# parthjaggi/flow

Measured on AMD Instinct MI355X. Metric: env-steps/sec, higher is better.
Workload: dtype mixed

## Files before the change

### flow_amd/csrc/flowsim_pair.h

```cpp
#pragma once
#include "flowsim_kernels.h"

namespace fs {

typedef float f2 __attribute__((ext_vector_type(2)));
typedef unsigned u2v __attribute__((__vector_size__(8)));

enum : int { DPP_ROW_NEWBCAST0 = 0x150, DPP_ROW_NEWBCAST8 = 0x158 };

__device__ __forceinline__ f2 fma2(f2 a, f2 b, f2 c) { return __builtin_elementwise_fma(a, b, c); }
__device__ __forceinline__ f2 splat(float a) { return f2{a, a}; }

__device__ __forceinline__ f2 pk_mul(f2 a, f2 b) { return a * b; }
__device__ __forceinline__ f2 pk_add(f2 a, f2 b) { return a + b; }
__device__ __forceinline__ f2 pk_sub(f2 a, f2 b) { return a - b; }
__device__ __forceinline__ f2 pk_fma(f2 a, f2 b, f2 c) { return fma2(a, b, c); }
__device__ __forceinline__ f2 pk_fnma(f2 a, f2 b, f2 c) { return fma2(-a, b, c); }
__device__ __forceinline__ float nonneg_else(float x, float y) {
  const unsigned a = __builtin_bit_cast(unsigned, x), b = __builtin_bit_cast(unsigned, y);
  return __builtin_bit_cast(float, min(a, b));
}

template <int ROW>
__device__ __forceinline__ float next_a(float v, bool last, int lane) {
// ... 70 lines not shown
  f2 adt, ddt;
};
template <bool FASTDIV>
__device__ __forceinline__ f2 sumo_acc_pair(f2 v, f2 vl, f2 h, const SumoPair& c, f2 one) {
  f2 gap;
  gap.x = tmax(h.x, 1e-3f);
  gap.y = tmax(h.y, 1e-3f);
  const f2 num = pk_mul(v, pk_sub(v, vl));
  const f2 dq = div_const2<FASTDIV>(num, c.ts, c.rc_ts);
  const f2 dyn = pk_add(pk_mul(v, c.tau), dq);
  f2 ss;
  ss.x = tmax(0.0f, dyn.x);
  ss.y = tmax(0.0f, dyn.y);
  ss = pk_add(c.min_gap, ss);
  const f2 q = FASTDIV ? div_core2(ss, gap, one) : f2{ss.x / gap.x, ss.y / gap.y};
  const f2 r = div_const2<FASTDIV>(v, c.smax, c.rc_smax);
  const f2 r2 = pk_mul(r, r);
  return pk_mul(c.maxa, pk_sub(pk_sub(one, pk_mul(r2, r2)), pk_mul(q, q)));
}

struct PairConsts {
  f2 p0, p1, p2, p5, rc_v0, tsab, rc_ab, one, dt2, ramp2, L2, rc_L2, len_lead, gap2, vmask, tvm;
  float c1e3;
  double ms64, rc_ms64;
  unsigned long long last_mask;
};
#define FS_PAIR_A_NAME pair_step_asm_a
#define FS_PAIR_A_NZ 0
#define FS_PAIR_A_NZ_PARAM
#include "flowsim_pair_step_a.inc"
#undef FS_PAIR_A_NAME
#undef FS_PAIR_A_NZ
#undef FS_PAIR_A_NZ_PARAM
#define FS_PAIR_A_NAME pair_step_asm_a_nz
#define FS_PAIR_A_NZ 1
#define FS_PAIR_A_NZ_PARAM , f2 nz
#include "flowsim_pair_step_a.inc"
#undef FS_PAIR_A_NAME
#undef FS_PAIR_A_NZ
#undef FS_PAIR_A_NZ_PARAM
#define FS_PAIR_A_NAME pair_step_asm_a_sm
#define FS_PAIR_A_NZ 0
#define FS_PAIR_A_NZ_PARAM
#include "flowsim_pair_step_a_sm.inc"
#undef FS_PAIR_A_NAME
#undef FS_PAIR_A_NZ
#undef FS_PAIR_A_NZ_PARAM
// ... 9 lines not shown
  asm volatile(
      "v_sub_f32_e32 v118, v112, v113\n"
      "v_sub_f32_e32 v132, v115, v114\n"
      "v_subrev_f32_dpp v119, v112, v113 row_shl:1 row_mask:0xf bank_mask:0xf bound_ctrl:1\n"
      "v_subrev_f32_dpp v134, v112, v113 row_newbcast:0 row_mask:0xf bank_mask:0xf\n"
      "v_sub_f32_dpp v133, v114, v115 row_shl:1 row_mask:0xf bank_mask:0xf bound_ctrl:1\n"
      "v_sub_f32_dpp v135, v114, v115 row_newbcast:0 row_mask:0xf bank_mask:0xf\n"
      "v_cndmask_b32_e64 v119, v119, v134, %[last]\n"
      "v_cndmask_b32_e64 v133, v133, v135, %[last]\n"
      "v_pk_add_f32 v[126:127], v[132:133], %[L2]\n"
      "v_min_u32_e32 v132, v132, v126\n"
      "v_min_u32_e32 v133, v133, v127\n"
      "v_pk_add_f32 v[116:117], v[132:133], %[lenlead] neg_lo:[0,1] neg_hi:[0,1]\n"
      "v_pk_add_f32 v[126:127], v[116:117], %[gap2] neg_lo:[0,1] neg_hi:[0,1]\n"
      "v_min_f32_e32 v126, v126, v127\n"
      "v_alignbit_b32 %[cb], %[cb], v126, 31\n"
      "v_pk_fma_f32 v[124:125], v[112:113], %[vmask], %[tvm]\n"
      "v_pk_mul_f32 v[124:125], v[124:125], v[124:125]\n"
      "v_add_f32_e32 %[sq], v124, v125\n"
      "v_cvt_f64_f32_e32 v[130:131], v112\n"
      "v_cvt_f64_f32_e32 v[132:133], v113\n"
      "v_mul_f64 v[134:135], v[130:131], %[rcms]\n"
      "v_mul_f64 v[136:137], v[132:133], %[rcms]\n"
      "v_fma_f64 v[130:131], -v[134:135], %[ms], v[130:131]\n"
      "v_fma_f64 v[132:133], -v[136:137], %[ms], v[132:133]\n"
      "v_fma_f64 v[134:135], v[130:131], %[rcms], v[134:135]\n"
      "v_fma_f64 v[136:137], v[132:133], %[rcms], v[136:137]\n"
      "v_cvt_f32_f64_e32 v128, v[134:135]\n"
      "v_cvt_f32_f64_e32 v129, v[136:137]\n"
      : "+{v[112:113]}"(V), "+{v[114:115]}"(X), "+{v[116:117]}"(H), "+{v[118:119]}"(DVL), "={v[128:129]}"(OV),
        [cb] "+v"(crash_bits), [sq] "=&v"(sq)
      : [L2] "v"(c.L2), [lenlead] "v"(c.len_lead), [gap2] "v"(c.gap2), [vmask] "v"(c.vmask), [tvm] "v"(c.tvm),
        [ms] "v"(c.ms64), [rcms] "v"(c.rc_ms64), [last] "s"(c.last_mask)
      : "v124", "v125", "v126", "v127", "v130", "v131", "v132", "v133", "v134", "v135", "v136", "v137");
}

struct MixedConsts {
  f2 p0, p1, p2, p5, rc_v0, tsab, rc_ab, one, gap2, vmask, tvm;
  float c1e3;
  double dt, ramp, L, rc_L, rc_ms, len_b, len_next, zero;
  unsigned L_lo, L_hi, thr;
  unsigned long long last_mask;
};
__device__ __forceinline__ void mixed_step_asm_a(f2& V32, double& XA, double& XB, double& VA, double& VB, f2& H, f2& DVL,
                                                 f2& OV, const MixedConsts& c) {
  asm volatile(
      "v_pk_mul_f32 v[124:125], v[112:113], v[142:143]\n"
      "v_pk_mul_f32 v[126:127], v[124:125], %[rcab]\n"
      "v_pk_fma_f32 v[130:131], v[126:127], %[tsab], v[124:125] neg_lo:[1,0,0] neg_hi:[1,0,0]\n"
      "v_pk_fma_f32 v[126:127], v[130:131], %[rcab], v[126:127]\n"
      "v_pk_mul_f32 v[124:125], v[112:113], %[rcv0]\n"
      "v_rcp_f32_e32 v122, v140\n"
      "v_rcp_f32_e32 v123, v141\n"
      "v_pk_fma_f32 v[130:131], v[124:125], %[p0], v[112:113] neg_lo:[1,0,0] neg_hi:[1,0,0]\n"
      "v_pk_fma_f32 v[124:125], v[130:131], %[rcv0], v[124:125]\n"
      "v_pk_mul_f32 v[130:131], v[112:113], %[p1]\n"
      "v_pk_add_f32 v[130:131], v[130:131], v[126:127]\n"
      "v_pk_fma_f32 v[126:127], v[140:141], v[122:123], %[one] neg_lo:[1,0,0] neg_hi:[1,0,0]\n"
      "v_max_f32_e32 v130, 0, v130\n"
      "v_max_f32_e32 v131, 0, v131\n"
      "v_pk_fma_f32 v[122:123], v[126:127], v[122:123], v[122:123]\n"
      "v_pk_add_f32 v[130:131], %[p5], v[130:131]\n"
      "v_pk_mul_f32 v[124:125], v[124:125], v[124:125]\n"
      "v_pk_mul_f32 v[126:127], v[130:131], v[122:123]\n"
      "v_pk_mul_f32 v[124:125], v[124:125], v[124:125]\n"
      "v_pk_fma_f32 v[132:133], v[140:141], v[126:127], v[130:131] neg_lo:[1,0,0] neg_hi:[1,0,0]\n"
      "v_pk_add_f32 v[124:125], %[one], v[124:125] neg_lo:[0,1] neg_hi:[0,1]\n"
      "v_pk_fma_f32 v[126:127], v[132:133], v[122:123], v[126:127]\n"
      "v_pk_fma_f32 v[132:133], v[140:141], v[126:127], v[130:131] neg_lo:[1,0,0] neg_hi:[1,0,0]\n"
      "v_pk_fma_f32 v[126:127], v[132:133], v[122:123], v[126:127]\n"
      "v_pk_mul_f32 v[126:127], v[126:127], v[126:127]\n"
      "v_pk_add_f32 v[124:125], v[124:125], v[126:127] neg_lo:[0,1] neg_hi:[0,1]\n"
      "v_pk_mul_f32 v[124:125], %[p2], v[124:125]\n"
      "v_cvt_f64_f32_e32 v[130:131], v124\n"
      "v_cvt_f64_f32_e32 v[132:133], v125\n"
      "v_mul_f64 v[130:131], v[130:131], %[dt]\n"
      "v_mul_f64 v[132:133], v[132:133], %[dt]\n"
      "v_add_f64 v[130:131], v[118:119], v[130:131]\n"
      "v_add_f64 v[132:133], v[138:139], v[132:133]\n"
      "v_max_f64 v[130:131], v[130:131], %[zero]\n"
      "v_max_f64 v[132:133], v[132:133], %[zero]\n"
      "v_add_f64 v[130:131], v[130:131], -v[118:119]\n"
      "v_add_f64 v[132:133], v[132:133], -v[138:139]\n"
      "v_mul_f64 v[130:131], v[130:131], %[ramp]\n"
      "v_mul_f64 v[132:133], v[132:133], %[ramp]\n"
      "v_add_f64 v[118:119], v[118:119], v[130:131]\n"
      "v_add_f64 v[138:139], v[138:139], v[132:133]\n"
      "v_cvt_f32_f64_e32 v112, v[118:119]\n"
      "v_cvt_f32_f64_e32 v113, v[138:139]\n"
      "v_mul_f64 v[130:131], v[118:119], %[dt]\n"
      "v_mul_f64 v[132:133], v[138:139], %[dt]\n"
      "v_add_f64 v[114:115], v[114:115], v[130:131]\n"
      "v_add_f64 v[116:117], v[116:117], v[132:133]\n"
      "v_mul_f64 v[120:121], v[118:119], %[rcms]\n"
      "v_mul_f64 v[122:123], v[138:139], %[rcms]\n"
      "v_cvt_f32_f64_e32 v128, v[120:121]\n"
      "v_cvt_f32_f64_e32 v129, v[122:123]\n"
      : "+{v[112:113]}"(V32), "+{v[114:115]}"(XA), "+{v[116:117]}"(XB), "+{v[118:119]}"(VA), "+{v[138:139]}"(VB),
        "+{v[140:141]}"(H), "+{v[142:143]}"(DVL), "={v[128:129]}"(OV)
      : [rcab] "v"(c.rc_ab), [tsab] "v"(c.tsab), [rcv0] "v"(c.rc_v0), [p0] "v"(c.p0), [p1] "v"(c.p1), [p2] "v"(c.p2),
        [p5] "v"(c.p5), [one] "v"(c.one), [dt] "v"(c.dt), [ramp] "v"(c.ramp), [rcms] "v"(c.rc_ms), [zero] "v"(c.zero)
      : "v120", "v121", "v122", "v123", "v124", "v125", "v126", "v127", "v130", "v131", "v132", "v133");
}
struct MixedSumoConsts { double fl0a, fl0b, adta, adtb, ddta, ddtb; };
__device__ __forceinline__ void mixed_step_asm_a_sm(f2& V32, double& XA, double& XB, double& VA, double& VB, f2& H,
                                                    f2& DVL, f2& OV, const MixedConsts& c, const SumoPair& m,
                                                    const MixedSumoConsts& d) {
  asm volatile(
      "v_pk_mul_f32 v[124:125], v[112:113], v[142:143]\n"
      "v_pk_mul_f32 v[126:127], v[124:125], %[rcab]\n"
      "v_pk_mul_f32 v[150:151], v[124:125], %[rcts]\n"
      "v_pk_fma_f32 v[130:131], v[126:127], %[tsab], v[124:125] neg_lo:[1,0,0] neg_hi:[1,0,0]\n"
      "v_pk_fma_f32 v[152:153], v[150:151], %[ts], v[124:125] neg_lo:[1,0,0] neg_hi:[1,0,0]\n"
      "v_pk_fma_f32 v[126:127], v[130:131], %[rcab], v[126:127]\n"
      "v_pk_fma_f32 v[150:151], v[152:153], %[rcts], v[150:151]\n"
      "v_max_f32_e32 v146, v140, %[c1e3]\n"
// ... 32 lines not shown
      "v_pk_fma_f32 v[134:135], v[146:147], v[152:153], v[150:151] neg_lo:[1,0,0] neg_hi:[1,0,0]\n"
      "v_pk_add_f32 v[124:125], %[one], v[124:125] neg_lo:[0,1] neg_hi:[0,1]\n"
      "v_pk_add_f32 v[154:155], %[one], v[154:155] neg_lo:[0,1] neg_hi:[0,1]\n"
      "v_pk_fma_f32 v[126:127], v[132:133], v[122:123], v[126:127]\n"
      "v_pk_fma_f32 v[152:153], v[134:135], v[148:149], v[152:153]\n"
      "v_pk_fma_f32 v[132:133], v[140:141], v[126:127], v[130:131] neg_lo:[1,0,0] neg_hi:[1,0,0]\n"
      "v_pk_fma_f32 v[134:135], v[146:147], v[152:153], v[150:151] neg_lo:[1,0,0] neg_hi:[1,0,0]\n"
      "v_pk_fma_f32 v[126:127], v[132:133], v[122:123], v[126:127]\n"
      "v_pk_fma_f32 v[152:153], v[134:135], v[148:149], v[152:153]\n"
      "v_pk_mul_f32 v[126:127], v[126:127], v[126:127]\n"
      "v_pk_mul_f32 v[152:153], v[152:153], v[152:153]\n"
      "v_pk_add_f32 v[124:125], v[124:125], v[126:127] neg_lo:[0,1] neg_hi:[0,1]\n"
      "v_pk_add_f32 v[154:155], v[154:155], v[152:153] neg_lo:[0,1] neg_hi:[0,1]\n"
      "v_pk_mul_f32 v[124:125], %[p2], v[124:125]\n"
      "v_pk_mul_f32 v[154:155], %[maxa], v[154:155]\n"
      "v_cvt_f64_f32_e32 v[130:131], v124\n"
      "v_cvt_f64_f32_e32 v[132:133], v125\n"
      "v_cvt_f64_f32_e32 v[134:135], v154\n"
      "v_cvt_f64_f32_e32 v[136:137], v155\n"
      "v_mul_f64 v[130:131], v[130:131], %[dt]\n"
      "v_mul_f64 v[132:133], v[132:133], %[dt]\n"
      "v_mul_f64 v[134:135], v[134:135], %[dt]\n"
      "v_mul_f64 v[136:137], v[136:137], %[dt]\n"
      "v_add_f64 v[130:131], v[118:119], v[130:131]\n"
      "v_add_f64 v[132:133], v[138:139], v[132:133]\n"
      "v_add_f64 v[134:135], v[118:119], v[134:135]\n"
      "v_add_f64 v[136:137], v[138:139], v[136:137]\n"
      "v_max_f64 v[130:131], v[130:131], %[zero]\n"
      "v_max_f64 v[132:133], v[132:133], %[zero]\n"
      "v_max_f64 v[134:135], v[134:135], %[fl0a]\n"
      "v_max_f64 v[136:137], v[136:137], %[fl0b]\n"
      "v_add_f64 v[130:131], v[130:131], -v[118:119]\n"
      "v_add_f64 v[132:133], v[132:133], -v[138:139]\n"
      "v_mul_f64 v[130:131], v[130:131], %[ramp]\n"
      "v_mul_f64 v[132:133], v[132:133], %[ramp]\n"
      "v_add_f64 v[130:131], v[118:119], v[130:131]\n"
      "v_add_f64 v[132:133], v[138:139], v[132:133]\n"
      "v_min_f64 v[130:131], v[130:131], v[134:135]\n"
      "v_min_f64 v[132:133], v[132:133], v[136:137]\n"
      "v_add_f64 v[134:135], v[118:119], %[adta]\n"
      "v_add_f64 v[136:137], v[138:139], %[adtb]\n"
      "v_min_f64 v[130:131], v[130:131], v[134:135]\n"
      "v_min_f64 v[132:133], v[132:133], v[136:137]\n"
      "v_add_f64 v[134:135], v[118:119], -%[ddta]\n"
      "v_add_f64 v[136:137], v[138:139], -%[ddtb]\n"
      "v_max_f64 v[118:119], v[130:131], v[134:135]\n"
      "v_max_f64 v[138:139], v[132:133], v[136:137]\n"
      "v_cvt_f32_f64_e32 v112, v[118:119]\n"
      "v_cvt_f32_f64_e32 v113, v[138:139]\n"
      "v_mul_f64 v[130:131], v[118:119], %[dt]\n"
      "v_mul_f64 v[132:133], v[138:139], %[dt]\n"
      "v_add_f64 v[114:115], v[114:115], v[130:131]\n"
      "v_add_f64 v[116:117], v[116:117], v[132:133]\n"
      "v_mul_f64 v[120:121], v[118:119], %[rcms]\n"
      "v_mul_f64 v[122:123], v[138:139], %[rcms]\n"
      "v_cvt_f32_f64_e32 v128, v[120:121]\n"
      "v_cvt_f32_f64_e32 v129, v[122:123]\n"
      : "+{v[112:113]}"(V32), "+{v[114:115]}"(XA), "+{v[116:117]}"(XB), "+{v[118:119]}"(VA), "+{v[138:139]}"(VB),
        "+{v[140:141]}"(H), "+{v[142:143]}"(DVL), "={v[128:129]}"(OV)
      : [c1e3] "v"(c.c1e3), [rcab] "v"(c.rc_ab), [tsab] "v"(c.tsab), [rcv0] "v"(c.rc_v0), [p0] "v"(c.p0),
        [p1] "v"(c.p1), [p2] "v"(c.p2), [p5] "v"(c.p5), [one] "v"(c.one), [dt] "v"(c.dt), [ramp] "v"(c.ramp),
        [rcms] "v"(c.rc_ms), [zero] "v"(c.zero), [rcts] "v"(m.rc_ts), [ts] "v"(m.ts),
        [rcsm] "v"(m.rc_smax), [smax] "v"(m.smax), [tau] "v"(m.tau), [mgap] "v"(m.min_gap), [maxa] "v"(m.maxa),
        [fl0a] "v"(d.fl0a), [fl0b] "v"(d.fl0b), [adta] "v"(d.adta), [adtb] "v"(d.adtb), [ddta] "v"(d.ddta),
        [ddtb] "v"(d.ddtb)
      : "v120", "v121", "v122", "v123", "v124", "v125", "v126", "v127", "v130", "v131", "v132", "v133", "v134",
        "v135", "v136", "v137", "v146", "v147", "v148", "v149", "v150", "v151", "v152", "v153", "v154", "v155");
}
__device__ __forceinline__ void mixed_step_asm_b(f2& V32, double& XA, double& XB, f2& H, f2& DVL, f2& OX, const double& WA,
                                                 const double& WB, float& ct, float& sq, unsigned long long& need,
                                                 const MixedConsts& c) {
  asm volatile(
      "v_sub_f32_e32 v142, v112, v113\n"
      "v_subrev_f32_dpp v143, v112, v113 row_shl:1 row_mask:0xf bank_mask:0xf bound_ctrl:1\n"
      "v_subrev_f32_dpp v124, v112, v113 row_newbcast:0 row_mask:0xf bank_mask:0xf\n"
      "v_mov_b32_dpp v130, v114 row_shl:1 row_mask:0xf bank_mask:0xf bound_ctrl:1\n"
      "v_mov_b32_dpp v131, v115 row_shl:1 row_mask:0xf bank_mask:0xf bound_ctrl:1\n"
      "v_mov_b32_dpp v132, v114 row_newbcast:0 row_mask:0xf bank_mask:0xf\n"
      "v_mov_b32_dpp v133, v115 row_newbcast:0 row_mask:0xf bank_mask:0xf\n"
      "v_add_f64 v[134:135], v[116:117], -v[114:115]\n"
      "v_cndmask_b32_e64 v130, v130, v132, %[last]\n"
      "v_cndmask_b32_e64 v131, v131, v133, %[last]\n"
      "v_add_f64 v[134:135], v[134:135], %[wa]\n"
      "v_add_f64 v[136:137], v[130:131], -v[116:117]\n"
      "v_cndmask_b32_e64 v143, v143, v124, %[last]\n"
      "v_add_f64 v[120:121], v[134:135], -%[lenb]\n"
      "v_add_f64 v[136:137], v[136:137], %[wb]\n"
      "v_max3_u32 v126, v115, v117, v135\n"
      "v_add_f64 v[122:123], v[136:137], -%[lennext]\n"
      "v_cvt_f32_f64_e32 v140, v[120:121]\n"
      "v_cvt_f32_f64_e32 v141, v[122:123]\n"
      "v_min_f32_e32 v127, v140, v141\n"
      "v_sub_u32_e32 v125, v127, %[c1e3]\n"
      "v_max3_u32 v126, v126, v137, v125\n"
      "v_cmp_le_u32_e64 %[need], %[thr], v126\n"
      "v_mul_f64 v[120:121], v[114:115], %[rcL]\n"
      "v_mul_f64 v[122:123], v[116:117], %[rcL]\n"
      "v_pk_fma_f32 v[124:125], v[112:113], %[vmask], %[tvm]\n"
      "v_cvt_f32_f64_e32 v144, v[120:121]\n"
      "v_cvt_f32_f64_e32 v145, v[122:123]\n"
      "v_pk_mul_f32 v[124:125], v[124:125], v[124:125]\n"
      "v_sub_f32_e32 %[ct], v127, %[gap]\n"
      "v_add_f32_e32 %[sq], v124, v125\n"
      : "+{v[112:113]}"(V32), "+{v[114:115]}"(XA), "+{v[116:117]}"(XB), "+{v[140:141]}"(H), "+{v[142:143]}"(DVL),
        "=&{v[144:145]}"(OX), [ct] "=&v"(ct), [sq] "=&v"(sq), [need] "=&s"(need)
      : [wa] "{v[156:157]}"(WA), [wb] "{v[158:159]}"(WB), [rcL] "v"(c.rc_L), [gap] "v"(c.gap2.x), [vmask] "v"(c.vmask), [tvm] "v"(c.tvm),
        [lenb] "v"(c.len_b), [lennext] "v"(c.len_next), [c1e3] "v"(c.c1e3), [thr] "v"(c.thr), [last] "s"(c.last_mask)
      : "v120", "v121", "v122", "v123", "v124", "v125", "v126", "v127", "v130", "v131", "v132", "v133", "v134", "v135",
        "v136", "v137");
}
__device__ __forceinline__ void mixed_step_asm_slow(double& XA, double& XB, f2& H, f2& OX, double& WA, double& WB, float& ct,
                                                    const MixedConsts& c) {
  unsigned long long sa, sb;
  asm volatile(
      "v_add_f64 v[134:135], v[114:115], -%[L]\n"
      "v_add_f64 v[136:137], v[116:117], -%[L]\n"
      "v_cmp_gt_i32_e64 %[sa], 0, v135\n"
      "v_cmp_gt_i32_e64 %[sb], 0, v137\n"
      "s_nop 0\n"
      "v_cndmask_b32_e64 v114, v134, v114, %[sa]\n"
      "v_cndmask_b32_e64 v115, v135, v115, %[sa]\n"
      "v_cndmask_b32_e64 v116, v136, v116, %[sb]\n"
      "v_cndmask_b32_e64 v117, v137, v117, %[sb]\n"
      "v_mul_f64 v[120:121], v[114:115], %[rcL]\n"
      "v_mul_f64 v[122:123], v[116:117], %[rcL]\n"
      "v_add_f64 v[134:135], v[116:117], -v[114:115]\n"
      "v_cvt_f32_f64_e32 v144, v[120:121]\n"
      "v_cvt_f32_f64_e32 v145, v[122:123]\n"
      "v_add_f64 v[126:127], v[134:135], %[L]\n"
      "v_mov_b32_dpp v130, v114 row_shl:1 row_mask:0xf bank_mask:0xf bound_ctrl:1\n"
      "v_mov_b32_dpp v131, v115 row_shl:1 row_mask:0xf bank_mask:0xf bound_ctrl:1\n"
      "v_mov_b32_dpp v132, v114 row_newbcast:0 row_mask:0xf bank_mask:0xf\n"
      "v_mov_b32_dpp v133, v115 row_newbcast:0 row_mask:0xf bank_mask:0xf\n"
      "v_cmp_gt_i32_e64 %[sa], 0, v135\n"
      "v_cndmask_b32_e64 v130, v130, v132, %[last]\n"
      "v_cndmask_b32_e64 v131, v131, v133, %[last]\n"
      "v_add_f64 v[136:137], v[130:131], -v[116:117]\n"
      "v_cndmask_b32_e64 v134, v134, v126, %[sa]\n"
      "v_cndmask_b32_e64 v135, v135, v127, %[sa]\n"
      "v_cndmask_b32_e64 v156, 0, %[Llo], %[sa]\n"
      "v_cndmask_b32_e64 v157, 0, %[Lhi], %[sa]\n"
      "v_add_f64 v[132:133], v[136:137], %[L]\n"
      "v_cmp_gt_i32_e64 %[sb], 0, v137\n"
      "v_add_f64 v[134:135], v[134:135], -%[lenb]\n"
      "v_cvt_f32_f64_e32 v140, v[134:135]\n"
      "v_cndmask_b32_e64 v136, v136, v132, %[sb]\n"
      "v_cndmask_b32_e64 v137, v137, v133, %[sb]\n"
      "v_cndmask_b32_e64 v158, 0, %[Llo], %[sb]\n"
      "v_cndmask_b32_e64 v159, 0, %[Lhi], %[sb]\n"
      "v_add_f64 v[136:137], v[136:137], -%[lennext]\n"
      "v_cvt_f32_f64_e32 v141, v[136:137]\n"
      "v_pk_add_f32 v[126:127], v[140:141], %[gap2] neg_lo:[0,1] neg_hi:[0,1]\n"
      "v_cmp_nlt_f32_e64 %[sa], |v140|, %[c1e3]\n"
      "v_cmp_nlt_f32_e64 %[sb], |v141|, %[c1e3]\n"
      "v_min_f32_e32 %[ct], v126, v127\n"
      "v_cndmask_b32_e64 v140, %[c1e3], v140, %[sa]\n"
      "v_cndmask_b32_e64 v141, %[c1e3], v141, %[sb]\n"
      : "+{v[114:115]}"(XA), "+{v[116:117]}"(XB), "+{v[140:141]}"(H), "+{v[144:145]}"(OX), "+{v[156:157]}"(WA),
        "+{v[158:159]}"(WB), [ct] "+v"(ct), [sa] "=&s"(sa), [sb] "=&s"(sb)
      : [L] "v"(c.L), [Llo] "v"(c.L_lo), [Lhi] "v"(c.L_hi), [rcL] "v"(c.rc_L), [gap2] "v"(c.gap2), [lenb] "v"(c.len_b),
        [lennext] "v"(c.len_next), [c1e3] "v"(c.c1e3), [last] "s"(c.last_mask)
      : "v120", "v121", "v122", "v123", "v126", "v127", "v130", "v131", "v132", "v133", "v134", "v135", "v136", "v137");
}

template <typename F, int... S>
__device__ __forceinline__ void each_slot(F&& f, std::integer_sequence<int, S...>) {
  (f(std::integral_constant<int, S>()), ...);
}

template <typename T, int ROW, bool DELTA4, bool FASTDIV, bool BADCHK, bool SM, bool NOISE, int NH>
__device__ __forceinline__ void rollout_pair_body(const DevView<T>& s, int num_steps, float* __restrict__ obs,
                                                  float* __restrict__ rew, uint8_t* __restrict__ done) {
  constexpr bool MIXED = sizeof(T) == 8;
  static_assert(!(NOISE && MIXED), "FS_MIXED has no noise form (its C twin cannot reproduce the hardware's log / cos)");
  constexpr bool ASM = ROW == 16 && DELTA4 && FASTDIV && !BADCHK;
  constexpr int RPW = 64 / ROW;
  constexpr int PERIOD = ROW < 16 ? ROW : 16;
  const int lane = threadIdx.x & 63;
  const int wave = (blockIdx.x * blockDim.x + threadIdx.x) >> 6;
  const int row = lane / ROW;
  const int k = lane % ROW;
  const int r = wave * RPW + row;
  const int N = NH > 0 ? 2 * NH : s.N;
  const int LP = N >> 1;
  const bool rvalid = r < s.R;
// ... 52 lines not shown

  auto headway = [&]() -> f2 {
    if (MIXED) {
      const double xn = next_a<ROW>(xdA, last, lane);
      double dA = xdB - xdA, dB = xn - xdB;
      dA = dA < 0.0 ? dA + L64 : dA;
      dB = dB < 0.0 ? dB + L64 : dB;
      return f2{float(dA - double(lenB)), float(dB - double(len_nextA))};
    } else {
      const f2 xl = {x.y, next_a<ROW>(x.x, last, lane)};
      f2 d = pk_sub(xl, x);
      const f2 dw = pk_add(d, L2);
      d.x = nonneg_else(d.x, dw.x);
      d.y = nonneg_else(d.y, dw.y);
      return pk_sub(d, len_lead);
    }
  };
  f2 h = headway();
  f2 vl = {v.y, next_a<ROW>(v.x, last, lane)};
  f2 dvl = v - vl;
  PairConsts pc;
  pc.p0 = p[0]; pc.p1 = p[1]; pc.p2 = p[2]; pc.p5 = p[5]; pc.rc_v0 = rc_v0; pc.tsab = two_sqrt_ab; pc.rc_ab = rc_ab;
  pc.one = one; pc.dt2 = dt2; pc.ramp2 = ramp2; pc.L2 = L2; pc.rc_L2 = rc_L2; pc.len_lead = len_lead;
  pc.gap2 = gap2; pc.vmask = vmask; pc.tvm = tvm; pc.c1e3 = 1e-3f; pc.ms64 = ms64; pc.rc_ms64 = rc_ms64;
  pc.last_mask = __ballot(last);
  MixedConsts mc;
  mc.p0 = p[0]; mc.p1 = p[1]; mc.p2 = p[2]; mc.p5 = p[5]; mc.rc_v0 = rc_v0; mc.tsab = two_sqrt_ab; mc.rc_ab = rc_ab;
  mc.one = one; mc.gap2 = gap2; mc.vmask = vmask; mc.tvm = tvm; mc.c1e3 = 1e-3f; mc.dt = dt64; mc.ramp = ramp64;
  mc.L = L64; mc.rc_L = rc_L64; mc.rc_ms = rc_ms64; mc.len_b = double(lenB); mc.len_next = double(len_nextA);
  mc.zero = 0.0; mc.last_mask = pc.last_mask;
  {
    const unsigned long long Lb = __builtin_bit_cast(unsigned long long, L64);
    mc.L_lo = unsigned(Lb); mc.L_hi = unsigned(Lb >> 32);
    mc.thr = mc.L_hi < 0x457CED91u ? mc.L_hi : 0x457CED91u;
  }
  double wA = 0.0, wB = 0.0;
  if constexpr (ASM && MIXED) {
    asm volatile("" : "+v"(mc.dt), "+v"(mc.ramp), "+v"(mc.one), "+v"(mc.zero), "+v"(mc.rc_ms), "+v"(mc.c1e3), "+v"(mc.gap2));
    const double xn = next_a<ROW>(xdA, last, lane);
    wA = xdB - xdA < 0.0 ? L64 : 0.0;
    wB = xn - xdB < 0.0 ? L64 : 0.0;
    h.x = tabs(h.x) < 1e-3f ? 1e-3f : h.x;
    h.y = tabs(h.y) < 1e-3f ? 1e-3f : h.y;
  }
  SumoPair sc{};
  double floor0A = 0, floor0B = 0, adtA = 0, adtB = 0, ddtA = 0, ddtB = 0;
  if constexpr (SM) {
    const int mA = s.speed_mode[iA], mB = s.speed_mode[iB];
    const float maA = float(s.max_accel[iA]), maB = float(s.max_accel[iB]);
    const float mdA = float(s.max_decel[iA]), mdB = float(s.max_decel[iB]);
    sc.tau = f2{float(s.sumo_tau[iA]), float(s.sumo_tau[iB])};
    sc.min_gap = f2{float(s.sumo_min_gap[iA]), float(s.sumo_min_gap[iB])};
    sc.maxa = f2{maA, maB};
    sc.smax = f2{float(s.sumo_max_speed[iA]), float(s.sumo_max_speed[iB])};
    sc.rc_smax = f2{1.0f / sc.smax.x, 1.0f / sc.smax.y};
    sc.ts = f2{2.0f * tsqrt(maA * mdA), 2.0f * tsqrt(maB * mdB)};
    sc.rc_ts = f2{1.0f / sc.ts.x, 1.0f / sc.ts.y};
    const float BIG = 3.0e38f;
    sc.floor0 = f2{(mA & 1) ? 0.0f : BIG, (mB & 1) ? 0.0f : BIG};
    sc.adt = f2{(mA & 2) ? maA * dt : BIG, (mB & 2) ? maB * dt : BIG};
    sc.ddt = f2{(mA & 4) ? mdA * dt : BIG, (mB & 4) ? mdB * dt : BIG};
// ... 85 lines not shown
    __builtin_amdgcn_fence(__ATOMIC_ACQUIRE, "wavefront");
  };

  auto noise_term = [&]() -> f2 {
    f2 nz = {-0.0f, -0.0f};
    if constexpr (NOISE) {
      const bool fresh = (nctr & 3u) == 0u;
      if (__ballot(fresh) != 0ull) {
        if (fresh) {
          gauss4<float>(s.seed_lo, s.seed_hi, s.rep0 + uint32_t(rr), uint32_t(iA), nctr >> 2, gA, s.noise_exact != 0);
          gauss4<float>(s.seed_lo, s.seed_hi, s.rep0 + uint32_t(rr), uint32_t(iB), nctr >> 2, gB, s.noise_exact != 0);
        }
      }
      const float tA = sigma.x * gA[0], tB = sigma.y * gB[0];
      nz.x = noisyA ? tA : -0.0f;
      nz.y = noisyB ? tB : -0.0f;
      gA[0] = gA[1]; gA[1] = gA[2]; gA[2] = gA[3];
      gB[0] = gB[1]; gB[1] = gB[2]; gB[2] = gB[3];
      nctr += 1u;
    }
    return nz;
  };

  auto one_step = [&](int slot, __amdgpu_buffer_rsrc_t rs, float& sq_out, auto IN_RING, __amdgpu_buffer_rsrc_t rs_prev)
                      __attribute__((always_inline)) {
    if constexpr (ASM) {
      f2 ov, ox;
      const unsigned so = unsigned(slot) * step_b32;
      auto store_late = [&]() {
        if constexpr (decltype(IN_RING)::value) {
          if (!BURST && slot >= 1 && slot <= NPIECE) __builtin_amdgcn_raw_buffer_store_b128(piece, rs_prev, doff[slot - 1], 0, 0);
        } else {
          if (slot > 0) __builtin_amdgcn_raw_buffer_store_b128(piece, rs, off_16, so - step_b32, 0);
        }
      };
      auto rows_in = [&]() {
        if constexpr (decltype(IN_RING)::value) ring_in(slot, ov, ox);
        else transpose_in(ov, ox);
      };
      if constexpr (MIXED) {
        if constexpr (SM) mixed_step_asm_a_sm(v, xdA, xdB, vdA, vdB, h, dvl, ov, mc, sc, msc);
        else mixed_step_asm_a(v, xdA, xdB, vdA, vdB, h, dvl, ov, mc);
        store_late();
        float ct;
        unsigned long long need;
        mixed_step_asm_b(v, xdA, xdB, h, dvl, ox, wA, wB, ct, sq_out, need, mc);
#if defined(FS_DIAG_ALWAYS_SLOW)
        need = ~0ull;
#elif defined(FS_DIAG_NEVER_SLOW)
        need = 0ull;
#endif
        if (__builtin_expect(need != 0ull, 0)) mixed_step_asm_slow(xdA, xdB, h, ox, wA, wB, ct, mc);
        crash_bits = __builtin_amdgcn_alignbit(crash_bits, __builtin_bit_cast(unsigned, ct), 31);
        rows_in();
      } else {
#if defined(FS_DIAG_NOSTORE)
        pair_step_asm_a(v, x, h, dvl, ox, pc);
        pair_step_asm_b(v, x, h, dvl, ov, crash_bits, sq_out, pc);
        asm volatile("" :: "v"(ov), "v"(ox), "s"(so));
#elif defined(FS_DIAG_NOXPOSE)
        pair_step_asm_a(v, x, h, dvl, ox, pc);
        __builtin_amdgcn_raw_buffer_store_b64(__builtin_bit_cast(u2v, ox), rs, off_x, so, 0);
        pair_step_asm_b(v, x, h, dvl, ov, crash_bits, sq_out, pc);
        __builtin_amdgcn_raw_buffer_store_b64(__builtin_bit_cast(u2v, ov), rs, off_v, so, 0);
#else
        if constexpr (NOISE) {
          const f2 nz = noise_term();
          if constexpr (SM) pair_step_asm_a_sm_nz(v, x, h, dvl, ox, pc, sc, nz);
          else pair_step_asm_a_nz(v, x, h, dvl, ox, pc, nz);
        } else {
          if constexpr (SM) pair_step_asm_a_sm(v, x, h, dvl, ox, pc, sc);
          else pair_step_asm_a(v, x, h, dvl, ox, pc);
        }
        store_late();
        pair_step_asm_b(v, x, h, dvl, ov, crash_bits, sq_out, pc);
        rows_in();
// ... 51 lines not shown
      const f2 vb = pk_sub(v, m100);
      bad_bits = __builtin_amdgcn_alignbit(bad_bits, __builtin_bit_cast(unsigned, __builtin_fminf(vb.x, vb.y)), 31);
    }
    f2 ov;
    if (MIXED) ov = f2{float(vdA * rc_ms64), float(vdB * rc_ms64)};
    else ov = f2{div_via_f64(v.x, ms64, rc_ms64), div_via_f64(v.y, ms64, rc_ms64)};
    const unsigned so = unsigned(slot) * step_b32;
    __builtin_amdgcn_raw_buffer_store_b64(__builtin_bit_cast(u2v, ov), rs, off_v, so, 0);
    __builtin_amdgcn_raw_buffer_store_b64(__builtin_bit_cast(u2v, ox), rs, off_x, so, 0);
    const f2 dv = pk_fma(v, vmask, tvm);
    const f2 sq = pk_mul(dv, dv);
    sq_out = sq.x + sq.y;
  };

  int base = 0;
  char* ob_prev = ob;
  unsigned prev_bytes = 0u;
  const std::integral_constant<bool, RING> in_ring{};
  for (; base + PERIOD <= num_steps; base += PERIOD) {
    float sq[PERIOD];
    const size_t remain = size_t(num_steps - base) * step_bytes;
    const __amdgpu_buffer_rsrc_t rs = __builtin_amdgcn_make_buffer_rsrc(
        ob, 0, remain > 0xFFFFFFFFull ? 0xFFFFFFFFu : unsigned(remain), 0x00020000);
    const __amdgpu_buffer_rsrc_t rs_prev = __builtin_amdgcn_make_buffer_rsrc(ob_prev, 0, prev_bytes, 0x00020000);
    if constexpr (RING) {
      each_slot([&](auto S) __attribute__((always_inline)) { one_step(S.value, rs, sq[S.value], in_ring, rs_prev); },
                std::make_integer_sequence<int, PERIOD>());
    } else {
#pragma unroll
      for (int slot = 0; slot < PERIOD; ++slot) one_step(slot, rs, sq[slot], in_ring, rs_prev);
    }
#if !defined(FS_DIAG_NOSTORE) && !defined(FS_DIAG_NOXPOSE)
    if constexpr (RING) {
      if constexpr (BURST) {
#pragma unroll
        for (int j = 0; j < NPIECE; ++j) __builtin_amdgcn_raw_buffer_store_b128(ring_piece(j), rs, doff[j], 0, 0);
        __builtin_amdgcn_fence(__ATOMIC_RELEASE, "wavefront");
        __builtin_amdgcn_wave_barrier();
        __builtin_amdgcn_fence(__ATOMIC_ACQUIRE, "wavefront");
      } else {
        ob_prev = ob;
        prev_bytes = unsigned(PERIOD) * step_b32;
      }
    } else if (XPOSE) {
      __builtin_amdgcn_raw_buffer_store_b128(piece, rs, off_16, unsigned(PERIOD - 1) * step_b32, 0);
    }
#endif
    ob += size_t(PERIOD) * step_bytes;
    tcount += PERIOD;
    const float racc = transposed_sum<ROW, PERIOD>(sq, lane);
    const unsigned crash_any = seg_or<ROW>(crash_bits);
    const unsigned bad_any = (BADCHK ? seg_or<ROW>(bad_bits) : 0u) | crash_any;
    crash_bits = 0u;
// ... 3 lines not shown
      const bool my_bad = (bad_any >> (PERIOD - 1 - k)) & 1u;
      const int t_k = tcount - (PERIOD - 1 - k);
      const float cost = tsqrt(racc);
      const float max_cost = float(s.max_cost);
      float reward = tmax(max_cost - cost, 0.0f) / (max_cost + 1.1920928955078125e-07f);
      reward = my_bad ? 0.0f : reward;
      const size_t o = size_t(base + k) * s.R + rr;
      rew[o] = reward;
      done[o] = done_flag(t_k >= s.step_limit, my_crash);
    }
  }
  if (RING && !BURST && prev_bytes != 0u) {
    const __amdgpu_buffer_rsrc_t rs_prev = __builtin_amdgcn_make_buffer_rsrc(ob_prev, 0, prev_bytes, 0x00020000);
#pragma unroll
    for (int j = 0; j < NPIECE; ++j) __builtin_amdgcn_raw_buffer_store_b128(ring_piece(j), rs_prev, doff[j], 0, 0);
    __builtin_amdgcn_fence(__ATOMIC_RELEASE, "wavefront");
    __builtin_amdgcn_wave_barrier();
    __builtin_amdgcn_fence(__ATOMIC_ACQUIRE, "wavefront");
  }
#pragma unroll 1
  for (; base < num_steps; ++base) {
    float sq1;
    const __amdgpu_buffer_rsrc_t rs = __builtin_amdgcn_make_buffer_rsrc(ob, 0, unsigned(step_bytes), 0x00020000);
    one_step(0, rs, sq1, std::false_type(), rs);
#if !defined(FS_DIAG_NOSTORE) && !defined(FS_DIAG_NOXPOSE)
    if (XPOSE) __builtin_amdgcn_raw_buffer_store_b128(piece, rs, off_16, 0u, 0);
#endif
    ob += step_bytes;
    tcount += 1;
    const float racc = seg_sum<ROW>(sq1);
    const bool my_crash = (seg_or<ROW>(crash_bits) & 1u) != 0u;
    const bool my_bad = (BADCHK && (seg_or<ROW>(bad_bits) & 1u) != 0u) || my_crash;
    crash_bits = 0u;
    bad_bits = 0u;
    if (rvalid && k == 0) {
      const float cost = tsqrt(racc);
      const float max_cost = float(s.max_cost);
      float reward = tmax(max_cost - cost, 0.0f) / (max_cost + 1.1920928955078125e-07f);
      reward = my_bad ? 0.0f : reward;
      const size_t o = size_t(base) * s.R + rr;
      rew[o] = reward;
      done[o] = done_flag(tcount >= s.step_limit, my_crash);
    }
  }
  if (valid) {
    if (MIXED) {
      s.pos[idx] = T(xdA); s.pos[idx + 1] = T(xdB);
// ... 37 lines not shown
```

Measured before the change: 15.07 billion.

## Fold crash test into slow-path gate and fuse f64 adds into FMAC

Replaces f64 add/fma instructions with two-operand v_fmac_f64 forms using inline 1.0/-1.0 constants and a precomputed negated max-speed, to shrink instruction encoding. In the fast mixed step, the per-step crash computation is removed and folded into the existing 'need slow path' threshold via a new ctest constant, so the crash bit is only computed and ORed in when the rare slow path runs. Slow-path SGPR masks are pinned to fixed registers and the ring's previous-pointer is kept in SGPRs. The changes risk subtle behaviour differences in crash detection thresholds (NaN handling, cap computation).

New measurement: 14.65 billion. 0.972x the previous value.

```diff
diff --git a/flow_amd/csrc/flowsim_pair.h b/flow_amd/csrc/flowsim_pair.h
--- a/flow_amd/csrc/flowsim_pair.h
+++ b/flow_amd/csrc/flowsim_pair.h
@@ -116,7 +116,7 @@
 struct PairConsts {
   f2 p0, p1, p2, p5, rc_v0, tsab, rc_ab, one, dt2, ramp2, L2, rc_L2, len_lead, gap2, vmask, tvm;
   float c1e3;
-  double ms64, rc_ms64;
+  double ms64, rc_ms64, nms64;
   unsigned long long last_mask;
 };
 #define FS_PAIR_A_NAME pair_step_asm_a
@@ -172,22 +172,22 @@
       "v_cvt_f64_f32_e32 v[132:133], v113\n"
       "v_mul_f64 v[134:135], v[130:131], %[rcms]\n"
       "v_mul_f64 v[136:137], v[132:133], %[rcms]\n"
-      "v_fma_f64 v[130:131], -v[134:135], %[ms], v[130:131]\n"
-      "v_fma_f64 v[132:133], -v[136:137], %[ms], v[132:133]\n"
-      "v_fma_f64 v[134:135], v[130:131], %[rcms], v[134:135]\n"
-      "v_fma_f64 v[136:137], v[132:133], %[rcms], v[136:137]\n"
+      "v_fmac_f64_e32 v[130:131], v[134:135], %[nms]\n"
+      "v_fmac_f64_e32 v[132:133], v[136:137], %[nms]\n"
+      "v_fmac_f64_e32 v[134:135], v[130:131], %[rcms]\n"
+      "v_fmac_f64_e32 v[136:137], v[132:133], %[rcms]\n"
       "v_cvt_f32_f64_e32 v128, v[134:135]\n"
       "v_cvt_f32_f64_e32 v129, v[136:137]\n"
       : "+{v[112:113]}"(V), "+{v[114:115]}"(X), "+{v[116:117]}"(H), "+{v[118:119]}"(DVL), "={v[128:129]}"(OV),
         [cb] "+v"(crash_bits), [sq] "=&v"(sq)
       : [L2] "v"(c.L2), [lenlead] "v"(c.len_lead), [gap2] "v"(c.gap2), [vmask] "v"(c.vmask), [tvm] "v"(c.tvm),
-        [ms] "v"(c.ms64), [rcms] "v"(c.rc_ms64), [last] "s"(c.last_mask)
+        [nms] "v"(c.nms64), [rcms] "v"(c.rc_ms64), [last] "s"(c.last_mask)
       : "v124", "v125", "v126", "v127", "v130", "v131", "v132", "v133", "v134", "v135", "v136", "v137");
 }
 
 struct MixedConsts {
   f2 p0, p1, p2, p5, rc_v0, tsab, rc_ab, one, gap2, vmask, tvm;
-  float c1e3;
+  float c1e3, ctest;
   double dt, ramp, L, rc_L, rc_ms, len_b, len_next, zero;
   unsigned L_lo, L_hi, thr;
   unsigned long long last_mask;
@@ -226,22 +226,22 @@
       "v_cvt_f64_f32_e32 v[132:133], v125\n"
       "v_mul_f64 v[130:131], v[130:131], %[dt]\n"
       "v_mul_f64 v[132:133], v[132:133], %[dt]\n"
-      "v_add_f64 v[130:131], v[118:119], v[130:131]\n"
-      "v_add_f64 v[132:133], v[138:139], v[132:133]\n"
+      "v_fmac_f64_e32 v[130:131], 1.0, v[118:119]\n"
+      "v_fmac_f64_e32 v[132:133], 1.0, v[138:139]\n"
       "v_max_f64 v[130:131], v[130:131], %[zero]\n"
       "v_max_f64 v[132:133], v[132:133], %[zero]\n"
-      "v_add_f64 v[130:131], v[130:131], -v[118:119]\n"
-      "v_add_f64 v[132:133], v[132:133], -v[138:139]\n"
+      "v_fmac_f64_e32 v[130:131], -1.0, v[118:119]\n"
+      "v_fmac_f64_e32 v[132:133], -1.0, v[138:139]\n"
       "v_mul_f64 v[130:131], v[130:131], %[ramp]\n"
       "v_mul_f64 v[132:133], v[132:133], %[ramp]\n"
-      "v_add_f64 v[118:119], v[118:119], v[130:131]\n"
-      "v_add_f64 v[138:139], v[138:139], v[132:133]\n"
+      "v_fmac_f64_e32 v[118:119], 1.0, v[130:131]\n"
+      "v_fmac_f64_e32 v[138:139], 1.0, v[132:133]\n"
       "v_cvt_f32_f64_e32 v112, v[118:119]\n"
       "v_cvt_f32_f64_e32 v113, v[138:139]\n"
       "v_mul_f64 v[130:131], v[118:119], %[dt]\n"
       "v_mul_f64 v[132:133], v[138:139], %[dt]\n"
-      "v_add_f64 v[114:115], v[114:115], v[130:131]\n"
-      "v_add_f64 v[116:117], v[116:117], v[132:133]\n"
+      "v_fmac_f64_e32 v[114:115], 1.0, v[130:131]\n"
+      "v_fmac_f64_e32 v[116:117], 1.0, v[132:133]\n"
       "v_mul_f64 v[120:121], v[118:119], %[rcms]\n"
       "v_mul_f64 v[122:123], v[138:139], %[rcms]\n"
       "v_cvt_f32_f64_e32 v128, v[120:121]\n"
@@ -320,20 +320,20 @@
       "v_mul_f64 v[132:133], v[132:133], %[dt]\n"
       "v_mul_f64 v[134:135], v[134:135], %[dt]\n"
       "v_mul_f64 v[136:137], v[136:137], %[dt]\n"
-      "v_add_f64 v[130:131], v[118:119], v[130:131]\n"
-      "v_add_f64 v[132:133], v[138:139], v[132:133]\n"
-      "v_add_f64 v[134:135], v[118:119], v[134:135]\n"
-      "v_add_f64 v[136:137], v[138:139], v[136:137]\n"
+      "v_fmac_f64_e32 v[130:131], 1.0, v[118:119]\n"
+      "v_fmac_f64_e32 v[132:133], 1.0, v[138:139]\n"
+      "v_fmac_f64_e32 v[134:135], 1.0, v[118:119]\n"
+      "v_fmac_f64_e32 v[136:137], 1.0, v[138:139]\n"
       "v_max_f64 v[130:131], v[130:131], %[zero]\n"
       "v_max_f64 v[132:133], v[132:133], %[zero]\n"
       "v_max_f64 v[134:135], v[134:135], %[fl0a]\n"
       "v_max_f64 v[136:137], v[136:137], %[fl0b]\n"
-      "v_add_f64 v[130:131], v[130:131], -v[118:119]\n"
-      "v_add_f64 v[132:133], v[132:133], -v[138:139]\n"
+      "v_fmac_f64_e32 v[130:131], -1.0, v[118:119]\n"
+      "v_fmac_f64_e32 v[132:133], -1.0, v[138:139]\n"
       "v_mul_f64 v[130:131], v[130:131], %[ramp]\n"
       "v_mul_f64 v[132:133], v[132:133], %[ramp]\n"
-      "v_add_f64 v[130:131], v[118:119], v[130:131]\n"
-      "v_add_f64 v[132:133], v[138:139], v[132:133]\n"
+      "v_fmac_f64_e32 v[130:131], 1.0, v[118:119]\n"
+      "v_fmac_f64_e32 v[132:133], 1.0, v[138:139]\n"
       "v_min_f64 v[130:131], v[130:131], v[134:135]\n"
       "v_min_f64 v[132:133], v[132:133], v[136:137]\n"
       "v_add_f64 v[134:135], v[118:119], %[adta]\n"
@@ -348,8 +348,8 @@
       "v_cvt_f32_f64_e32 v113, v[138:139]\n"
       "v_mul_f64 v[130:131], v[118:119], %[dt]\n"
       "v_mul_f64 v[132:133], v[138:139], %[dt]\n"
-      "v_add_f64 v[114:115], v[114:115], v[130:131]\n"
-      "v_add_f64 v[116:117], v[116:117], v[132:133]\n"
+      "v_fmac_f64_e32 v[114:115], 1.0, v[130:131]\n"
+      "v_fmac_f64_e32 v[116:117], 1.0, v[132:133]\n"
       "v_mul_f64 v[120:121], v[118:119], %[rcms]\n"
       "v_mul_f64 v[122:123], v[138:139], %[rcms]\n"
       "v_cvt_f32_f64_e32 v128, v[120:121]\n"
@@ -366,7 +366,7 @@
         "v135", "v136", "v137", "v146", "v147", "v148", "v149", "v150", "v151", "v152", "v153", "v154", "v155");
 }
 __device__ __forceinline__ void mixed_step_asm_b(f2& V32, double& XA, double& XB, f2& H, f2& DVL, f2& OX, const double& WA,
-                                                 const double& WB, float& ct, float& sq, unsigned long long& need,
+                                                 const double& WB, float& sq, unsigned long long& need,
                                                  const MixedConsts& c) {
   asm volatile(
       "v_sub_f32_e32 v142, v112, v113\n"
@@ -379,47 +379,44 @@
       "v_add_f64 v[134:135], v[116:117], -v[114:115]\n"
       "v_cndmask_b32_e64 v130, v130, v132, %[last]\n"
       "v_cndmask_b32_e64 v131, v131, v133, %[last]\n"
-      "v_add_f64 v[134:135], v[134:135], %[wa]\n"
-      "v_add_f64 v[136:137], v[130:131], -v[116:117]\n"
+      "v_fmac_f64_e32 v[134:135], 1.0, v[156:157]\n"
+      "v_fmac_f64_e32 v[130:131], -1.0, v[116:117]\n"
+      "v_fmac_f64_e32 v[130:131], 1.0, v[158:159]\n"
+      "v_max3_u32 v126, v115, v135, v131\n"
+      "v_fmac_f64_e32 v[134:135], -1.0, %[lenb]\n"
+      "v_fmac_f64_e32 v[130:131], -1.0, %[lennext]\n"
+      "v_cvt_f32_f64_e32 v140, v[134:135]\n"
+      "v_cvt_f32_f64_e32 v141, v[130:131]\n"
+      "v_min_f32_e32 v127, v140, v141\n"
+      "v_sub_u32_e32 v125, v127, %[ctest]\n"
+      "v_max3_u32 v126, v126, v117, v125\n"
+      "v_cmp_le_u32_e64 %[need], %[thr], v126\n"
       "v_cndmask_b32_e64 v143, v143, v124, %[last]\n"
-      "v_add_f64 v[120:121], v[134:135], -%[lenb]\n"
-      "v_add_f64 v[136:137], v[136:137], %[wb]\n"
-      "v_max3_u32 v126, v115, v117, v135\n"
-      "v_add_f64 v[122:123], v[136:137], -%[lennext]\n"
-      "v_cvt_f32_f64_e32 v140, v[120:121]\n"
-      "v_cvt_f32_f64_e32 v141, v[122:123]\n"
-      "v_min_f32_e32 v127, v140, v141\n"
-      "v_sub_u32_e32 v125, v127, %[c1e3]\n"
-      "v_max3_u32 v126, v126, v137, v125\n"
-      "v_cmp_le_u32_e64 %[need], %[thr], v126\n"
       "v_mul_f64 v[120:121], v[114:115], %[rcL]\n"
       "v_mul_f64 v[122:123], v[116:117], %[rcL]\n"
       "v_pk_fma_f32 v[124:125], v[112:113], %[vmask], %[tvm]\n"
       "v_cvt_f32_f64_e32 v144, v[120:121]\n"
       "v_cvt_f32_f64_e32 v145, v[122:123]\n"
       "v_pk_mul_f32 v[124:125], v[124:125], v[124:125]\n"
-      "v_sub_f32_e32 %[ct], v127, %[gap]\n"
       "v_add_f32_e32 %[sq], v124, v125\n"
       : "+{v[112:113]}"(V32), "+{v[114:115]}"(XA), "+{v[116:117]}"(XB), "+{v[140:141]}"(H), "+{v[142:143]}"(DVL),
-        "=&{v[144:145]}"(OX), [ct] "=&v"(ct), [sq] "=&v"(sq), [need] "=&s"(need)
-      : [wa] "{v[156:157]}"(WA), [wb] "{v[158:159]}"(WB), [rcL] "v"(c.rc_L), [gap] "v"(c.gap2.x), [vmask] "v"(c.vmask), [tvm] "v"(c.tvm),
-        [lenb] "v"(c.len_b), [lennext] "v"(c.len_next), [c1e3] "v"(c.c1e3), [thr] "v"(c.thr), [last] "s"(c.last_mask)
-      : "v120", "v121", "v122", "v123", "v124", "v125", "v126", "v127", "v130", "v131", "v132", "v133", "v134", "v135",
-        "v136", "v137");
-}
-__device__ __forceinline__ void mixed_step_asm_slow(double& XA, double& XB, f2& H, f2& OX, double& WA, double& WB, float& ct,
+        "=&{v[144:145]}"(OX), [sq] "=&v"(sq), [need] "={s[96:97]}"(need)
+      : "{v[156:157]}"(WA), "{v[158:159]}"(WB), [rcL] "v"(c.rc_L), [vmask] "v"(c.vmask), [tvm] "v"(c.tvm),
+        [lenb] "v"(c.len_b), [lennext] "v"(c.len_next), [ctest] "v"(c.ctest), [thr] "v"(c.thr), [last] "s"(c.last_mask)
+      : "v120", "v121", "v122", "v123", "v124", "v125", "v126", "v127", "v130", "v131", "v132", "v133", "v134", "v135");
+}
+__device__ __forceinline__ void mixed_step_asm_slow(double& XA, double& XB, f2& H, f2& OX, double& WA, double& WB, unsigned& ct,
                                                     const MixedConsts& c) {
-  unsigned long long sa, sb;
   asm volatile(
       "v_add_f64 v[134:135], v[114:115], -%[L]\n"
       "v_add_f64 v[136:137], v[116:117], -%[L]\n"
-      "v_cmp_gt_i32_e64 %[sa], 0, v135\n"
-      "v_cmp_gt_i32_e64 %[sb], 0, v137\n"
+      "v_cmp_gt_i32_e64 s[98:99], 0, v135\n"
+      "v_cmp_gt_i32_e64 s[100:101], 0, v137\n"
       "s_nop 0\n"
-      "v_cndmask_b32_e64 v114, v134, v114, %[sa]\n"
-      "v_cndmask_b32_e64 v115, v135, v115, %[sa]\n"
-      "v_cndmask_b32_e64 v116, v136, v116, %[sb]\n"
-      "v_cndmask_b32_e64 v117, v137, v117, %[sb]\n"
+      "v_cndmask_b32_e64 v114, v134, v114, s[98:99]\n"
+      "v_cndmask_b32_e64 v115, v135, v115, s[98:99]\n"
+      "v_cndmask_b32_e64 v116, v136, v116, s[100:101]\n"
+      "v_cndmask_b32_e64 v117, v137, v117, s[100:101]\n"
       "v_mul_f64 v[120:121], v[114:115], %[rcL]\n"
       "v_mul_f64 v[122:123], v[116:117], %[rcL]\n"
       "v_add_f64 v[134:135], v[116:117], -v[114:115]\n"
@@ -430,35 +427,37 @@
       "v_mov_b32_dpp v131, v115 row_shl:1 row_mask:0xf bank_mask:0xf bound_ctrl:1\n"
       "v_mov_b32_dpp v132, v114 row_newbcast:0 row_mask:0xf bank_mask:0xf\n"
       "v_mov_b32_dpp v133, v115 row_newbcast:0 row_mask:0xf bank_mask:0xf\n"
-      "v_cmp_gt_i32_e64 %[sa], 0, v135\n"
+      "v_cmp_gt_i32_e64 s[98:99], 0, v135\n"
       "v_cndmask_b32_e64 v130, v130, v132, %[last]\n"
       "v_cndmask_b32_e64 v131, v131, v133, %[last]\n"
-      "v_add_f64 v[136:137], v[130:131], -v[116:117]\n"
-      "v_cndmask_b32_e64 v134, v134, v126, %[sa]\n"
-      "v_cndmask_b32_e64 v135, v135, v127, %[sa]\n"
-      "v_cndmask_b32_e64 v156, 0, %[Llo], %[sa]\n"
-      "v_cndmask_b32_e64 v157, 0, %[Lhi], %[sa]\n"
-      "v_add_f64 v[132:133], v[136:137], %[L]\n"
-      "v_cmp_gt_i32_e64 %[sb], 0, v137\n"
-      "v_add_f64 v[134:135], v[134:135], -%[lenb]\n"
+      "v_fmac_f64_e32 v[130:131], -1.0, v[116:117]\n"
+      "v_cndmask_b32_e64 v134, v134, v126, s[98:99]\n"
+      "v_cndmask_b32_e64 v135, v135, v127, s[98:99]\n"
+      "v_cndmask_b32_e64 v156, 0, %[Llo], s[98:99]\n"
+      "v_cndmask_b32_e64 v157, 0, %[Lhi], s[98:99]\n"
+      "v_add_f64 v[132:133], v[130:131], %[L]\n"
+      "v_cmp_gt_i32_e64 s[100:101], 0, v131\n"
+      "v_fmac_f64_e32 v[134:135], -1.0, %[lenb]\n"
       "v_cvt_f32_f64_e32 v140, v[134:135]\n"
-      "v_cndmask_b32_e64 v136, v136, v132, %[sb]\n"
-      "v_cndmask_b32_e64 v137, v137, v133, %[sb]\n"
-      "v_cndmask_b32_e64 v158, 0, %[Llo], %[sb]\n"
-      "v_cndmask_b32_e64 v159, 0, %[Lhi], %[sb]\n"
-      "v_add_f64 v[136:137], v[136:137], -%[lennext]\n"
-      "v_cvt_f32_f64_e32 v141, v[136:137]\n"
+      "v_cndmask_b32_e64 v130, v130, v132, s[100:101]\n"
+      "v_cndmask_b32_e64 v131, v131, v133, s[100:101]\n"
+      "v_cndmask_b32_e64 v158, 0, %[Llo], s[100:101]\n"
+      "v_cndmask_b32_e64 v159, 0, %[Lhi], s[100:101]\n"
+      "v_fmac_f64_e32 v[130:131], -1.0, %[lennext]\n"
+      "v_cvt_f32_f64_e32 v141, v[130:131]\n"
       "v_pk_add_f32 v[126:127], v[140:141], %[gap2] neg_lo:[0,1] neg_hi:[0,1]\n"
-      "v_cmp_nlt_f32_e64 %[sa], |v140|, %[c1e3]\n"
-      "v_cmp_nlt_f32_e64 %[sb], |v141|, %[c1e3]\n"
+      "v_cmp_nlt_f32_e64 s[98:99], |v140|, %[c1e3]\n"
+      "v_cmp_nlt_f32_e64 s[100:101], |v141|, %[c1e3]\n"
       "v_min_f32_e32 %[ct], v126, v127\n"
-      "v_cndmask_b32_e64 v140, %[c1e3], v140, %[sa]\n"
-      "v_cndmask_b32_e64 v141, %[c1e3], v141, %[sb]\n"
+      "v_cndmask_b32_e64 v140, %[c1e3], v140, s[98:99]\n"
+      "v_cndmask_b32_e64 v141, %[c1e3], v141, s[100:101]\n"
+      "v_lshrrev_b32_e32 %[ct], 31, %[ct]\n"
       : "+{v[114:115]}"(XA), "+{v[116:117]}"(XB), "+{v[140:141]}"(H), "+{v[144:145]}"(OX), "+{v[156:157]}"(WA),
-        "+{v[158:159]}"(WB), [ct] "+v"(ct), [sa] "=&s"(sa), [sb] "=&s"(sb)
+        "+{v[158:159]}"(WB), [ct] "=&v"(ct)
       : [L] "v"(c.L), [Llo] "v"(c.L_lo), [Lhi] "v"(c.L_hi), [rcL] "v"(c.rc_L), [gap2] "v"(c.gap2), [lenb] "v"(c.len_b),
         [lennext] "v"(c.len_next), [c1e3] "v"(c.c1e3), [last] "s"(c.last_mask)
-      : "v120", "v121", "v122", "v123", "v126", "v127", "v130", "v131", "v132", "v133", "v134", "v135", "v136", "v137");
+      : "v120", "v121", "v122", "v123", "v126", "v127", "v130", "v131", "v132", "v133", "v134", "v135", "v136", "v137",
+        "s98", "s99", "s100", "s101");
 }
 
 template <typename F, int... S>
@@ -557,21 +556,24 @@
   PairConsts pc;
   pc.p0 = p[0]; pc.p1 = p[1]; pc.p2 = p[2]; pc.p5 = p[5]; pc.rc_v0 = rc_v0; pc.tsab = two_sqrt_ab; pc.rc_ab = rc_ab;
   pc.one = one; pc.dt2 = dt2; pc.ramp2 = ramp2; pc.L2 = L2; pc.rc_L2 = rc_L2; pc.len_lead = len_lead;
-  pc.gap2 = gap2; pc.vmask = vmask; pc.tvm = tvm; pc.c1e3 = 1e-3f; pc.ms64 = ms64; pc.rc_ms64 = rc_ms64;
+  pc.gap2 = gap2; pc.vmask = vmask; pc.tvm = tvm; pc.c1e3 = 1e-3f; pc.ms64 = ms64; pc.rc_ms64 = rc_ms64; pc.nms64 = -ms64;
   pc.last_mask = __ballot(last);
   MixedConsts mc;
   mc.p0 = p[0]; mc.p1 = p[1]; mc.p2 = p[2]; mc.p5 = p[5]; mc.rc_v0 = rc_v0; mc.tsab = two_sqrt_ab; mc.rc_ab = rc_ab;
   mc.one = one; mc.gap2 = gap2; mc.vmask = vmask; mc.tvm = tvm; mc.c1e3 = 1e-3f; mc.dt = dt64; mc.ramp = ramp64;
+  mc.ctest = gap2.x > 1e-3f ? gap2.x : 1e-3f;
   mc.L = L64; mc.rc_L = rc_L64; mc.rc_ms = rc_ms64; mc.len_b = double(lenB); mc.len_next = double(len_nextA);
   mc.zero = 0.0; mc.last_mask = pc.last_mask;
   {
     const unsigned long long Lb = __builtin_bit_cast(unsigned long long, L64);
     mc.L_lo = unsigned(Lb); mc.L_hi = unsigned(Lb >> 32);
-    mc.thr = mc.L_hi < 0x457CED91u ? mc.L_hi : 0x457CED91u;
+    const unsigned cap = 0x80000000u - __builtin_bit_cast(unsigned, mc.ctest);
+    mc.thr = mc.L_hi < cap ? mc.L_hi : cap;
+    if (!(gap2.x == gap2.x)) mc.thr = 0u;
   }
   double wA = 0.0, wB = 0.0;
   if constexpr (ASM && MIXED) {
-    asm volatile("" : "+v"(mc.dt), "+v"(mc.ramp), "+v"(mc.one), "+v"(mc.zero), "+v"(mc.rc_ms), "+v"(mc.c1e3), "+v"(mc.gap2));
+    asm volatile("" : "+v"(mc.dt), "+v"(mc.ramp), "+v"(mc.one), "+v"(mc.zero), "+v"(mc.rc_ms), "+v"(mc.c1e3), "+v"(mc.ctest), "+v"(mc.gap2));
     const double xn = next_a<ROW>(xdA, last, lane);
     wA = xdB - xdA < 0.0 ? L64 : 0.0;
     wB = xn - xdB < 0.0 ? L64 : 0.0;
@@ -703,8 +705,8 @@
     return nz;
   };
 
-  auto one_step = [&](int slot, __amdgpu_buffer_rsrc_t rs, float& sq_out, auto IN_RING, __amdgpu_buffer_rsrc_t rs_prev)
-                      __attribute__((always_inline)) {
+  auto one_step = [&](int slot, __amdgpu_buffer_rsrc_t rs, float& sq_out, auto IN_RING, __amdgpu_buffer_rsrc_t rs_prev,
+                      int cbit) __attribute__((always_inline)) {
     if constexpr (ASM) {
       f2 ov, ox;
       const unsigned so = unsigned(slot) * step_b32;
@@ -723,16 +725,18 @@
         if constexpr (SM) mixed_step_asm_a_sm(v, xdA, xdB, vdA, vdB, h, dvl, ov, mc, sc, msc);
         else mixed_step_asm_a(v, xdA, xdB, vdA, vdB, h, dvl, ov, mc);
         store_late();
-        float ct;
         unsigned long long need;
-        mixed_step_asm_b(v, xdA, xdB, h, dvl, ox, wA, wB, ct, sq_out, need, mc);
+        mixed_step_asm_b(v, xdA, xdB, h, dvl, ox, wA, wB, sq_out, need, mc);
 #if defined(FS_DIAG_ALWAYS_SLOW)
         need = ~0ull;
 #elif defined(FS_DIAG_NEVER_SLOW)
         need = 0ull;
 #endif
-        if (__builtin_expect(need != 0ull, 0)) mixed_step_asm_slow(xdA, xdB, h, ox, wA, wB, ct, mc);
-        crash_bits = __builtin_amdgcn_alignbit(crash_bits, __builtin_bit_cast(unsigned, ct), 31);
+        if (__builtin_expect(need != 0ull, 0)) {
+          unsigned ct;
+          mixed_step_asm_slow(xdA, xdB, h, ox, wA, wB, ct, mc);
+          crash_bits |= ct << cbit;
+        }
         rows_in();
       } else {
 #if defined(FS_DIAG_NOSTORE)
@@ -830,13 +834,15 @@
     const size_t remain = size_t(num_steps - base) * step_bytes;
     const __amdgpu_buffer_rsrc_t rs = __builtin_amdgcn_make_buffer_rsrc(
         ob, 0, remain > 0xFFFFFFFFull ? 0xFFFFFFFFu : unsigned(remain), 0x00020000);
-    const __amdgpu_buffer_rsrc_t rs_prev = __builtin_amdgcn_make_buffer_rsrc(ob_prev, 0, prev_bytes, 0x00020000);
+    char* ob_prev_here = ob_prev;
+    if constexpr (RING) asm volatile("" : "+s"(ob_prev_here));
+    const __amdgpu_buffer_rsrc_t rs_prev = __builtin_amdgcn_make_buffer_rsrc(ob_prev_here, 0, prev_bytes, 0x00020000);
     if constexpr (RING) {
-      each_slot([&](auto S) __attribute__((always_inline)) { one_step(S.value, rs, sq[S.value], in_ring, rs_prev); },
+      each_slot([&](auto S) __attribute__((always_inline)) { one_step(S.value, rs, sq[S.value], in_ring, rs_prev, PERIOD - 1 - S.value); },
                 std::make_integer_sequence<int, PERIOD>());
     } else {
 #pragma unroll
-      for (int slot = 0; slot < PERIOD; ++slot) one_step(slot, rs, sq[slot], in_ring, rs_prev);
+      for (int slot = 0; slot < PERIOD; ++slot) one_step(slot, rs, sq[slot], in_ring, rs_prev, PERIOD - 1 - slot);
     }
 #if !defined(FS_DIAG_NOSTORE) && !defined(FS_DIAG_NOXPOSE)
     if constexpr (RING) {
@@ -886,7 +892,7 @@
   for (; base < num_steps; ++base) {
     float sq1;
     const __amdgpu_buffer_rsrc_t rs = __builtin_amdgcn_make_buffer_rsrc(ob, 0, unsigned(step_bytes), 0x00020000);
-    one_step(0, rs, sq1, std::false_type(), rs);
+    one_step(0, rs, sq1, std::false_type(), rs, 0);
 #if !defined(FS_DIAG_NOSTORE) && !defined(FS_DIAG_NOXPOSE)
     if (XPOSE) __builtin_amdgcn_raw_buffer_store_b128(piece, rs, off_16, 0u, 0);
 #endif
```
